# LioQing/wgpu-3dgs-core

Measured on AMD Instinct MI355X. Metric: Msplats/s @1080p (Gaussians per second through proj+sort+blend; 3 frames in flight on 3 priority streams), higher is better.
Workload: dtype f32; 1 GPU; 1M synthetic Gaussians, SH degree 0 (ShNone/RotScale 48 B), 1920x1080; gaussians=1000000, visible=708615, pairs=2550276, launches_per_frame=14, parallelism=single GPU, 3 frames in flight on 3 priority streams, frames_in_flight=3, renderer_scratch_copies=3

## Files before the change

### wgpu-3dgs-core_amd/csrc/gs_render_kernels.h

```cpp
#pragma once

#include <type_traits>

#include "gs_device_common.h"

namespace gs {

constexpr int PP_THREADS = 256;
constexpr int PP_ITEMS = 4;
constexpr int PP_CHUNK = PP_THREADS * PP_ITEMS;

struct FrameConsts {
    float M[16];
    float V[16];
    float ISR[9];
    float WS[9];
    float cam_pos[3];
    float fx, fy, cx, cy;
    float near_plane, far_plane;
    float size2, limx, limy, max_std_dev;
    float bg[3];
    uint32_t sh_deg, no_sh0;
    uint32_t width, height;
    uint32_t tiles_x, tiles_y;
// ... 2964 lines not shown
    if (wid == 0u) {
        blend_tile_range(tk, ranges, tile, lane, true, start, end);
        if (lane == 0u) {
            s_range[0] = start;
            s_range[1] = end;
        }
    }
    __syncthreads();
    start = s_range[0];
    end = s_range[1];
}

constexpr int BLEND_THREADS = 128;
constexpr int BLEND_BATCH = 128;

template <int MODE>
__global__ __launch_bounds__(BLEND_THREADS) void k_blend(uint32_t *__restrict__ ranges,
                                                         const uint32_t *__restrict__ idx,
                                                         const uint32_t *__restrict__ recs,
                                                         FrameConsts fc, float4 *__restrict__ rgba,
                                                         const FrameState *__restrict__ state, TileKeys tk) {
    if (state->overflow) return;
    __shared__ float4 s_a[2][BLEND_BATCH];
    __shared__ float4 s_b[2][BLEND_BATCH];
    __shared__ float2 s_c[2][BLEND_BATCH];
    __shared__ uint32_t s_cnt[2][2];
    __shared__ uint32_t s_alive[2];

    const uint32_t tid = threadIdx.x, lane = tid & 63u, wid = tid >> 6;
    const uint32_t tile = fc.band_ty0 * fc.tiles_x + blockIdx.x;
    const uint32_t ty = tile / fc.tiles_x, tx = tile % fc.tiles_x;
    const uint32_t px = tx * 16u + (lane & 15u);
    const uint32_t py0 = ty * 16u + wid * 8u + (lane >> 4), py1 = py0 + 4u;
    const float pxf = (float)px + 0.5f;
    const float rx0 = (float)(tx * 16u) + 0.5f, rx1 = rx0 + 15.0f;
    const float ry0 = (float)(ty * 16u) + 0.5f;

    uint32_t start, end;
    __shared__ uint32_t s_range[2];
    blend_tile_range_wg(tk, ranges, tile, lane, wid, s_range, start, end);
    f32x2 T = {1.0f, 1.0f}, C0 = {0.0f, 0.0f}, C1 = {0.0f, 0.0f}, C2 = {0.0f, 0.0f};
    const bool in0 = px < fc.width && py0 < fc.height, in1 = px < fc.width && py1 < fc.height;
    constexpr float DEAD = 1.0e15f;
    f32x2 pyf = {in0 ? (float)py0 + 0.5f : DEAD, in1 ? (float)py1 + 0.5f : DEAD};
    uint32_t remaining = __builtin_amdgcn_readfirstlane(
        (uint32_t)__popcll(__ballot(in0)) + (uint32_t)__popcll(__ballot(in1)));

    for (uint32_t b0 = start; b0 < end; b0 += BLEND_BATCH) {
        if (lane == 0) s_alive[wid] = remaining;
        __syncthreads();
        if ((s_alive[0] | s_alive[1]) == 0u) break;

        uint32_t j = b0 + tid;
        bool keep0 = false, keep1 = false;
        float pmin = 0.0f;
        u32x4_a4 r0, r1;
        uint32_t r2x = 0;
        if (j < end) {
            const uint32_t *rec = recs + (uint64_t)idx[j] * REC_WORDS;
            r0 = *(const u32x4_a4 *)(rec);
            r1 = *(const u32x4_a4 *)(rec + 4);
            r2x = rec[8];
            float mx = u2f(r0.x), my = u2f(r0.y), ca = u2f(r0.z), cb = u2f(r0.w), cc = u2f(r1.x);
            if constexpr (MODE == 0) {
                pmin = fmaxf(-__logf(255.0f * u2f(r1.y)) - 1.0e-3f, -5.6f);
                const float thr = (pmin - 0.1f) - cull_rounding_slack(mx, my, ca, cb, cc, rx0, ry0);
                keep0 = splat_touches_rect(mx, my, ca, cb, cc, rx0, rx1, ry0, ry0 + 7.0f, thr);
                keep1 = splat_touches_rect(mx, my, ca, cb, cc, rx0, rx1, ry0 + 8.0f, ry0 + 15.0f, thr);
            } else if constexpr (MODE == 1) {
                pmin = fc.ellipse_pmin;
                const float thr = (pmin - 0.1f - 1.0e-3f * fabsf(pmin)) - cull_rounding_slack(mx, my, ca, cb, cc, rx0, ry0);
                keep0 = splat_touches_rect(mx, my, ca, cb, cc, rx0, rx1, ry0, ry0 + 7.0f, thr);
                keep1 = splat_touches_rect(mx, my, ca, cb, cc, rx0, rx1, ry0 + 8.0f, ry0 + 15.0f, thr);
            } else {
                const float ex = mx - clampf(mx, rx0, rx1);
                const float ey0 = my - clampf(my, ry0, ry0 + 7.0f), ey1 = my - clampf(my, ry0 + 8.0f, ry0 + 15.0f);
                keep0 = ex * ex + ey0 * ey0 <= 2.26f;
                keep1 = ex * ex + ey1 * ey1 <= 2.26f;
            }
        }
        uint64_t m0 = __ballot(keep0), m1 = __ballot(keep1);
        if (lane == 0) {
            s_cnt[wid][0] = (uint32_t)__popcll(m0);
            s_cnt[wid][1] = (uint32_t)__popcll(m1);
        }
        __syncthreads();
        const uint32_t base0 = wid ? s_cnt[0][0] : 0u, base1 = wid ? s_cnt[0][1] : 0u;
        const uint32_t kept =
            __builtin_amdgcn_readfirstlane(s_cnt[0][wid] + s_cnt[1][wid]);
        if (keep0) {
            uint32_t pos = base0 + mbcnt(m0);
            s_a[0][pos] = make_float4(u2f(r0.x), u2f(r0.y), u2f(r0.z), u2f(r0.w));
            s_b[0][pos] = make_float4(u2f(r1.x), u2f(r1.y), u2f(r1.z), u2f(r1.w));
            s_c[0][pos] = make_float2(u2f(r2x), pmin);
        }
        if (keep1) {
            uint32_t pos = base1 + mbcnt(m1);
            s_a[1][pos] = make_float4(u2f(r0.x), u2f(r0.y), u2f(r0.z), u2f(r0.w));
            s_b[1][pos] = make_float4(u2f(r1.x), u2f(r1.y), u2f(r1.z), u2f(r1.w));
            s_c[1][pos] = make_float2(u2f(r2x), pmin);
        }
        __syncthreads();

        if (remaining != 0u) {
            for (uint32_t s = 0; s < kept; s++) {
                const float4 a = s_a[wid][s];
                const float4 bq = s_b[wid][s];
                const float dx = a.x - pxf;
                const f32x2 dy = f32x2{a.y, a.y} - pyf;
                const float u = a.z * dx, wq = a.w * dx;
                const f32x2 v = f32x2{bq.x, bq.x} * dy;
                f32x2 t = f32x2{wq, wq} * dy;
                t = pk_fma(v, dy, t);
                const f32x2 power = pk_fma(f32x2{u, u}, f32x2{dx, dx}, t);
                const float2 cq = s_c[wid][s];
                bool p0, p1;
                if constexpr (MODE == 2) {
                    const f32x2 d2 = f32x2{dx * dx, dx * dx} + dy * dy;
                    p0 = d2.x <= 2.25f;
                    p1 = d2.y <= 2.25f;
                } else {
                    p0 = power.x <= 0.0f && power.x >= cq.y;
                    p1 = power.y <= 0.0f && power.y >= cq.y;
                }
                if (!__any(p0 || p1)) continue;
                f32x2 alpha;
                if constexpr (MODE == 0) {
                const f32x2 tt = power * f32x2{1.44269504088896340736f, 1.44269504088896340736f};
                const f32x2 tm = tt + f32x2{12582912.0f, 12582912.0f};
                const f32x2 n = tm - f32x2{12582912.0f, 12582912.0f};
                const f32x2 f = tt - n;
                f32x2 p = {0x1.5f0896p-10f, 0x1.5f0896p-10f};
                p = pk_fma(p, f, f32x2{0x1.3cbf6cp-7f, 0x1.3cbf6cp-7f});
                p = pk_fma(p, f, f32x2{0x1.c6af6cp-5f, 0x1.c6af6cp-5f});
                p = pk_fma(p, f, f32x2{0x1.ebfa4ap-3f, 0x1.ebfa4ap-3f});
                p = pk_fma(p, f, f32x2{0x1.62e430p-1f, 0x1.62e430p-1f});
                p = pk_fma(p, f, f32x2{1.0f, 1.0f});
                const f32x2 e = {u2f(f2u(p.x) + (f2u(tm.x) << 23)), u2f(f2u(p.y) + (f2u(tm.y) << 23))};
                const f32x2 oe = f32x2{bq.y, bq.y} * e;
                alpha = f32x2{fminf(0.99f, oe.x), fminf(0.99f, oe.y)};
                } else {
                    const float flat = fminf(0.99f, bq.y);
                    alpha = f32x2{flat, flat};
                }
                const bool act0 = p0 && alpha.x >= (1.0f / 255.0f);
                const bool act1 = p1 && alpha.y >= (1.0f / 255.0f);
                f32x2 alpha_eff = {act0 ? alpha.x : 0.0f, act1 ? alpha.y : 0.0f};
                f32x2 test_T = T * (f32x2{1.0f, 1.0f} - alpha_eff);
                const bool fin0 = act0 && test_T.x < 0.0001f, fin1 = act1 && test_T.y < 0.0001f;
                if (__any(fin0 || fin1)) {
                    if (fin0) { pyf.x = DEAD; alpha_eff.x = 0.0f; test_T.x = T.x; }
                    if (fin1) { pyf.y = DEAD; alpha_eff.y = 0.0f; test_T.y = T.y; }
                    remaining = __builtin_amdgcn_readfirstlane(
                        remaining - ((uint32_t)__popcll(__ballot(fin0)) + (uint32_t)__popcll(__ballot(fin1))));
                }
                const f32x2 wgt = alpha_eff * T;
                C0 = pk_fma(f32x2{bq.z, bq.z}, wgt, C0);
                C1 = pk_fma(f32x2{bq.w, bq.w}, wgt, C1);
                C2 = pk_fma(f32x2{cq.x, cq.x}, wgt, C2);
                T = test_T;
                if (remaining == 0u) break;
            }
        }
    }
    if (in0) {
        float4 o;
        o.x = __builtin_fmaf(T.x, fc.bg[0], C0.x);
        o.y = __builtin_fmaf(T.x, fc.bg[1], C1.x);
        o.z = __builtin_fmaf(T.x, fc.bg[2], C2.x);
        o.w = 1.0f - T.x;
        store16(rgba + (uint64_t)py0 * fc.width + px, make_uint4(f2u(o.x), f2u(o.y), f2u(o.z), f2u(o.w)), fc.wt_stores);
    }
    if (in1) {
        float4 o;
        o.x = __builtin_fmaf(T.y, fc.bg[0], C0.y);
        o.y = __builtin_fmaf(T.y, fc.bg[1], C1.y);
        o.z = __builtin_fmaf(T.y, fc.bg[2], C2.y);
        o.w = 1.0f - T.y;
        store16(rgba + (uint64_t)py1 * fc.width + px, make_uint4(f2u(o.x), f2u(o.y), f2u(o.z), f2u(o.w)), fc.wt_stores);
    }
}


__device__ __forceinline__ bool splat_touches_rect2(float mx, float my, float ca, float cb, float cc,
                                                    float rx0, float rx1, float ry0, float ry1, float thr) {
    const float dx_lo = mx - rx1, dx_hi = mx - rx0, dy_lo = my - ry1, dy_hi = my - ry0;
    const bool in_x = dx_lo <= 0.0f && dx_hi >= 0.0f, in_y = dy_lo <= 0.0f && dy_hi >= 0.0f;
    const float dxn = fabsf(dx_lo) < fabsf(dx_hi) ? dx_lo : dx_hi;
    const float dyn = fabsf(dy_lo) < fabsf(dy_hi) ? dy_lo : dy_hi;
    const float mv = parabola_max(cc, cb * dxn, ca * dxn * dxn, dy_lo, dy_hi);
    const float mh = parabola_max(ca, cb * dyn, cc * dyn * dyn, dx_lo, dx_hi);
    return (in_x && in_y) || !(fmaxf(mv, mh) < thr);
}

constexpr uint32_t PICK_NONE = 0xffffffffu;
struct AuxIO {
    float *depth;
    uint32_t *pick;
    float tcut;
    uint32_t key_bias;
    const uint32_t *depth_keys;
    const uint32_t *block_list;
    const uint32_t *order;
};
__device__ __forceinline__ uint32_t aux_caller_index(const AuxIO &aux, uint32_t slot) {
    if (slot == PICK_NONE) return PICK_NONE;
    if (aux.block_list) slot = aux.block_list[slot / (uint32_t)PP_CHUNK] * (uint32_t)PP_CHUNK + slot % (uint32_t)PP_CHUNK;
    return aux.order ? aux.order[slot] : slot;
}
__device__ __forceinline__ void store4(void *p, uint32_t v, uint32_t mode) {
    if (mode == 1u) asm volatile("global_store_dword %0, %1, off sc1" ::"v"(p), "v"(v) : "memory");
    else if (mode == 2u) asm volatile("global_store_dword %0, %1, off nt" ::"v"(p), "v"(v) : "memory");
    else if (mode == 3u) asm volatile("global_store_dword %0, %1, off sc0 sc1" ::"v"(p), "v"(v) : "memory");
    else *(uint32_t *)p = v;
}
__device__ __forceinline__ void aux_store(const AuxIO &aux, uint64_t pix, uint32_t depth_bits, uint32_t pick, uint32_t mode) {
    if (aux.depth) store4(aux.depth + pix, depth_bits, mode);
    if (aux.pick) store4(aux.pick + pix, pick, mode);
}

__device__ __forceinline__ AuxIO aux_io() { return AuxIO{}; }
__device__ __forceinline__ AuxIO aux_io(AuxIO a) { return a; }

struct ContribIO {
    uint4 *rec;
    const uint32_t *block_list;
    const uint32_t *order;
};
__device__ __forceinline__ AuxIO aux_io(ContribIO) { return AuxIO{}; }
__device__ __forceinline__ ContribIO contrib_io() { return ContribIO{}; }
__device__ __forceinline__ ContribIO contrib_io(AuxIO) { return ContribIO{}; }
__device__ __forceinline__ ContribIO contrib_io(ContribIO c) { return c; }
template <typename... A> struct is_contrib_pack : std::false_type {};
template <> struct is_contrib_pack<ContribIO> : std::true_type {};
__device__ __forceinline__ uint32_t contrib_caller_index(const ContribIO &c, uint32_t slot) {
    if (c.block_list) slot = c.block_list[slot / (uint32_t)PP_CHUNK] * (uint32_t)PP_CHUNK + slot % (uint32_t)PP_CHUNK;
    return c.order ? c.order[slot] : slot;
}
template <int OFF> __device__ __forceinline__ uint32_t contrib_other_half(uint32_t v) {
    static_assert(OFF == 1 || OFF == 2 || OFF == 4 || OFF == 8 || OFF == 16, "inside a group of at most 32 lanes");
    if constexpr (OFF == 1) return (uint32_t)__builtin_amdgcn_update_dpp(0, (int)v, 0xB1, 0xf, 0xf, true);
    else if constexpr (OFF == 2) return (uint32_t)__builtin_amdgcn_update_dpp(0, (int)v, 0x4E, 0xf, 0xf, true);
    else if constexpr (OFF == 4) return (uint32_t)__builtin_amdgcn_update_dpp(0, (int)v, 0x141, 0xf, 0xf, true);
    else if constexpr (OFF == 8) return (uint32_t)__builtin_amdgcn_update_dpp(0, (int)v, 0x140, 0xf, 0xf, true);
    else return (uint32_t)__builtin_amdgcn_ds_swizzle((int)v, 0x401F);
}
template <int GL>
__device__ __forceinline__ void contrib_add(unsigned long long *s_qh, uint32_t *s_max, uint32_t acc, float w0, float w1, uint32_t lg) {
    uint32_t q = (uint32_t)(w0 * 16777216.0f) + (uint32_t)(w1 * 16777216.0f);
    uint32_t h = (w0 > 0.0f ? 1u : 0u) + (w1 > 0.0f ? 1u : 0u);
    uint32_t m = f2u(w0) > f2u(w1) ? f2u(w0) : f2u(w1);
#define GS_CONTRIB_FOLD(OFF)                                  \
    if constexpr (GL > OFF) {                                 \
        const uint32_t oq = contrib_other_half<OFF>(q);       \
        const uint32_t oh = contrib_other_half<OFF>(h);       \
        const uint32_t om = contrib_other_half<OFF>(m);       \
        q += oq;                                              \
        h += oh;                                              \
        m = om > m ? om : m;                                  \
    }
    GS_CONTRIB_FOLD(1)
    GS_CONTRIB_FOLD(2)
    GS_CONTRIB_FOLD(4)
    GS_CONTRIB_FOLD(8)
    GS_CONTRIB_FOLD(16)
#undef GS_CONTRIB_FOLD
    if (lg == 0u && h != 0u) {
        (void)__hip_atomic_fetch_add((unsigned long long *)((char *)s_qh + 2u * acc), ((unsigned long long)h << 32) | q, __ATOMIC_RELAXED,
                                     __HIP_MEMORY_SCOPE_WORKGROUP);
        (void)__hip_atomic_fetch_max((uint32_t *)((char *)s_max + acc), m, __ATOMIC_RELAXED, __HIP_MEMORY_SCOPE_WORKGROUP);
    }
}
__device__ __forceinline__ void contrib_flush(const ContribIO &c, uint32_t index, unsigned long long qh, uint32_t m) {
    if ((uint32_t)(qh >> 32) != 0u) {
        uint4 *p = c.rec + index;
        (void)__hip_atomic_fetch_add((unsigned long long *)p, qh & 0xffffffffull, __ATOMIC_RELAXED, __HIP_MEMORY_SCOPE_AGENT);
        (void)__hip_atomic_fetch_add((uint32_t *)p + 2, (uint32_t)(qh >> 32), __ATOMIC_RELAXED, __HIP_MEMORY_SCOPE_AGENT);
        (void)__hip_atomic_fetch_max((uint32_t *)p + 3, m, __ATOMIC_RELAXED, __HIP_MEMORY_SCOPE_AGENT);
    }
}

template <int MODE, int G, bool ROUNDS = false, bool AUX = false, typename... AuxArg>
__global__ __launch_bounds__(BLEND_THREADS) void k_blend_grouped(uint32_t *__restrict__ ranges,
                                                                 const uint32_t *__restrict__ idx,
                                                                 const uint32_t *__restrict__ recs,
                                                                 FrameConsts fc, float4 *__restrict__ rgba,
                                                                 const FrameState *__restrict__ state, TileKeys tk,
                                                                 AuxArg... aux_arg) {
    constexpr bool CONTRIB = is_contrib_pack<AuxArg...>::value;
    static_assert(sizeof...(AuxArg) == (AUX || CONTRIB ? 1u : 0u), "the AUX blend takes one AuxIO, the CONTRIB one one ContribIO, the plain one none");
    static_assert(!CONTRIB || (!AUX && !ROUNDS), "contribution frames take one round and no planes");
    static_assert(G == 2 || G == 4 || G == 8, "lane groups per wave");
    if (state->overflow) return;
    constexpr int GL = WAVE / G;
    constexpr int BW = G == 8 ? 4 : 8;
    constexpr int BH = 2 * GL / BW;
    constexpr int NCOL = 16 / BW;
    constexpr int NROW = 16 / BH;
    constexpr int NL = 2 * G;
    static_assert(NCOL * NROW == NL && G == NCOL * (NROW / 2), "one list per block, G blocks per wave");
    constexpr uint32_t NULL_REC = BLEND_BATCH;
    constexpr uint32_t RS = 48;
    __shared__ __attribute__((aligned(16))) float s_rec[(BLEND_BATCH + 1) * (RS / 4)];
    __shared__ __attribute__((aligned(16))) uint16_t s_list_mem[NL * BLEND_BATCH + (G == 8 ? 2 : 0)];
    uint16_t(*const s_list)[BLEND_BATCH] = (uint16_t(*)[BLEND_BATCH])s_list_mem;
    typedef typename std::conditional<G == 8, uint16_t, uint32_t>::type cnt_t;
    __shared__ __attribute__((aligned(16))) cnt_t s_cnt[2][NL];
    __shared__ uint32_t s_alive[2];

    const uint32_t tid = threadIdx.x, lane = tid & 63u, wid = tid >> 6;
    const uint32_t tile = fc.band_ty0 * fc.tiles_x + blockIdx.x;
    const uint32_t ty = tile / fc.tiles_x, tx = tile % fc.tiles_x;
    const uint32_t gi = lane / GL, lg = lane % GL;
    const uint32_t bx = gi % (uint32_t)NCOL, by = gi / (uint32_t)NCOL;
    const uint32_t px = tx * 16u + bx * (uint32_t)BW + lg % (uint32_t)BW;
    const uint32_t py0 = ty * 16u + wid * 8u + by * BH + lg / (uint32_t)BW, py1 = py0 + BH / 2;
    const float pxf = (float)px + 0.5f;
    const uint32_t my_list = wid * G + gi;
    const float tx0 = (float)(tx * 16u) + 0.5f, ty0 = (float)(ty * 16u) + 0.5f;

    if (ROUNDS && tk.round == 2u && ((tk.done[tile >> 5] >> (tile & 31u)) & 1u)) return;
    uint32_t start, end;
    __shared__ uint32_t s_range[2];
    __shared__ uint32_t s_limit[MODE == 0 ? 256 : 1];
    if constexpr (MODE == 0) {
        s_limit[tid] = k_blend_np_limit[tid];
        s_limit[tid + BLEND_THREADS] = k_blend_np_limit[tid + BLEND_THREADS];
    }
    blend_tile_range_wg(tk, ranges, tile, lane, wid, s_range, start, end);
    f32x2 T = {1.0f, 1.0f}, C0 = {0.0f, 0.0f}, C1 = {0.0f, 0.0f}, C2 = {0.0f, 0.0f};
    const bool in0 = px < fc.width && py0 < fc.height, in1 = px < fc.width && py1 < fc.height;
    constexpr float DEAD = 1.0e15f;
    bool live0 = in0, live1 = in1;
    if (ROUNDS && tk.round == 2u) {
        if (in0) {
            const float4 s = rgba[(uint64_t)py0 * fc.width + px];
            C0.x = s.x; C1.x = s.y; C2.x = s.z; T.x = fabsf(s.w);
            live0 = s.w > 0.0f;
        }
        if (in1) {
            const float4 s = rgba[(uint64_t)py1 * fc.width + px];
            C0.y = s.x; C1.y = s.y; C2.y = s.z; T.y = fabsf(s.w);
            live1 = s.w > 0.0f;
        }
    }
    f32x2 D = {0.0f, 0.0f};
    uint32_t pk0 = PICK_NONE, pk1 = PICK_NONE;
    const AuxIO aux = aux_io(aux_arg...);
    const ContribIO cio = contrib_io(aux_arg...);
    unsigned long long *s_qh = nullptr;
    uint32_t *s_max = nullptr;
    uint32_t my_index = 0u;
    bool flush_pending = false;
    if constexpr (CONTRIB) {
        __shared__ __attribute__((aligned(8))) unsigned long long s_contrib_qh[BLEND_BATCH];
        __shared__ uint32_t s_contrib_max[BLEND_BATCH];
        s_qh = s_contrib_qh;
        s_max = s_contrib_max;
    }
    if (AUX && ROUNDS && tk.round == 2u) {
        if (in0) {
            if (aux.depth) D.x = aux.depth[(uint64_t)py0 * fc.width + px];
            if (aux.pick) pk0 = aux.pick[(uint64_t)py0 * fc.width + px];
        }
        if (in1) {
            if (aux.depth) D.y = aux.depth[(uint64_t)py1 * fc.width + px];
            if (aux.pick) pk1 = aux.pick[(uint64_t)py1 * fc.width + px];
        }
    }
    f32x2 pyf = {live0 ? (float)py0 + 0.5f : DEAD, live1 ? (float)py1 + 0.5f : DEAD};
    uint32_t remaining = __builtin_amdgcn_readfirstlane(
        (uint32_t)__popcll(__ballot(live0)) + (uint32_t)__popcll(__ballot(live1)));
    if (tid == 0) {
        *(float4 *)(s_rec + NULL_REC * (RS / 4)) = make_float4(0.0f, 0.0f, 0.0f, 0.0f);
        *(float4 *)(s_rec + NULL_REC * (RS / 4) + 4) = make_float4(0.0f, MODE == 2 ? 1.0f : 0.0f, 0.0f, 0.0f);
        if constexpr (AUX || CONTRIB) *(float4 *)(s_rec + NULL_REC * (RS / 4) + 8) = make_float4(0.0f, 0.0f, 0.0f, 0.0f);
        else *(float2 *)(s_rec + NULL_REC * (RS / 4) + 8) = make_float2(0.0f, 0.0f);
    }

    for (uint32_t b0 = start; b0 < end; b0 += BLEND_BATCH) {
        if (lane == 0) s_alive[wid] = remaining;
        __syncthreads();
        if constexpr (CONTRIB) {
            if (flush_pending) contrib_flush(cio, my_index, s_qh[tid], s_max[tid]);
            flush_pending = false;
        }
        if ((s_alive[0] | s_alive[1]) == 0u) break;

        if constexpr (G == 8) {
            uint4 *l128 = (uint4 *)&s_list[0][0];
            constexpr uint32_t fill = (NULL_REC * RS) * 0x00010001u;
#pragma unroll
            for (uint32_t q = 0; q < NL * BLEND_BATCH / 8; q += BLEND_THREADS) l128[q + tid] = make_uint4(fill, fill, fill, fill);
        } else {
            uint32_t *l32 = (uint32_t *)&s_list[0][0];
            constexpr uint32_t fill = (NULL_REC * RS) * 0x00010001u;
            for (uint32_t q = tid; q < NL * BLEND_BATCH / 2; q += BLEND_THREADS) l32[q] = fill;
        }
        const uint32_t j = b0 + tid;
        float mx = 0.0f, my = 0.0f, ca = 0.0f, cb = 0.0f, cc = 0.0f, thr = 0.0f;
        uint32_t limit = 0u;
        const bool have = j < end;
        const bool staging = __builtin_amdgcn_ballot_w64(have) != 0ull;
        if constexpr (CONTRIB) {
            s_qh[tid] = 0ull;
            s_max[tid] = 0u;
        }
        uint64_t m[NL];
        if (!staging) {
#pragma unroll
            for (int l = 0; l < NL; l++) m[l] = 0ull;
        } else {
            if (have) {
                const uint32_t slot = idx[j];
                const uint32_t *rec = recs + (uint64_t)slot * REC_WORDS;
                const u32x4_a4 r0 = *(const u32x4_a4 *)(rec);
                const u32x4_a4 r1 = *(const u32x4_a4 *)(rec + 4);
                const uint32_t r2x = rec[8];
                mx = u2f(r0.x); my = u2f(r0.y); ca = u2f(r0.z); cb = u2f(r0.w); cc = u2f(r1.x);
                float pmin;
                if constexpr (MODE == 0) {
                    limit = s_limit[(uint32_t)(255.0f * u2f(r1.y) + 0.5f) & 255u];
                    pmin = fminf(-u2f(limit - 1u), 0.0f);
                } else {
                    pmin = fc.ellipse_pmin;
                    limit = f2u(fabsf(pmin)) + 1u;
                }
                thr = (MODE == 0 ? pmin : pmin - 1.0e-3f * fabsf(pmin)) - cull_rounding_slack(mx, my, ca, cb, cc, tx0, ty0);
                *(float4 *)(s_rec + tid * (RS / 4)) = make_float4(mx, my, ca, cb);
                *(float4 *)(s_rec + tid * (RS / 4) + 4) = make_float4(cc, MODE == 2 ? pmin : u2f(limit), u2f(r1.y), u2f(r1.z));
                if constexpr (AUX)
                    *(float4 *)(s_rec + tid * (RS / 4) + 8) =
                        make_float4(u2f(r1.w), u2f(r2x), u2f(aux.depth_keys[slot] + aux.key_bias), u2f(slot));
                else if constexpr (CONTRIB) {
                    *(float4 *)(s_rec + tid * (RS / 4) + 8) = make_float4(u2f(r1.w), u2f(r2x), 0.0f, u2f(tid * 4u));
                    my_index = contrib_caller_index(cio, slot);
                }
                else
                    *(float2 *)(s_rec + tid * (RS / 4) + 8) = make_float2(u2f(r1.w), u2f(r2x));
            }
            float bx0 = tx0, by0 = ty0;
            if constexpr (G == 8) asm volatile("" : "+v"(bx0), "+v"(by0));
            if constexpr (MODE == 2) {
#pragma unroll
                for (int l = 0; l < NL; l++) {
                    const int lw = l / G, lgi = l % G;
                    const float rx0 = bx0 + (float)BW * (float)(lgi % NCOL);
                    const float ry0 = by0 + 8.0f * (float)lw + (float)BH * (float)(lgi / NCOL);
                    const float ex = mx - clampf(mx, rx0, rx0 + (float)(BW - 1)), ey = my - clampf(my, ry0, ry0 + (float)(BH - 1));
                    m[l] = __builtin_amdgcn_ballot_w64(have && ex * ex + ey * ey <= 2.26f);
                }
            } else {
                const float rcc = __builtin_amdgcn_rcpf(cc), rca = __builtin_amdgcn_rcpf(ca);
                float c_lo[NCOL], c_hi[NCOL], c_q1[NCOL], c_q0[NCOL], c_t[NCOL];
                uint64_t c_inb[NCOL];
                const uint64_t have_b = __builtin_amdgcn_ballot_w64(have && limit != 0u);
#pragma unroll
                for (int c = 0; c < NCOL; c++) {
                    const float x0c = bx0 + (float)BW * (float)c;
                    c_lo[c] = mx - (x0c + (float)(BW - 1));
                    c_hi[c] = mx - x0c;
                    c_inb[c] = __builtin_amdgcn_ballot_w64(c_lo[c] <= 0.0f) & __builtin_amdgcn_ballot_w64(c_hi[c] >= 0.0f);
                    const float dn = fabsf(c_lo[c]) < fabsf(c_hi[c]) ? c_lo[c] : c_hi[c];
                    c_q1[c] = cb * dn;
                    c_q0[c] = ca * dn * dn;
                    c_t[c] = -0.5f * c_q1[c] * rcc;
                }
#pragma unroll
                for (int r = 0; r < NROW; r++) {
                    const float y0r = by0 + (float)(BH * r);
                    const float r_lo = my - (y0r + (float)(BH - 1)), r_hi = my - y0r;
                    const uint64_t r_inb = __builtin_amdgcn_ballot_w64(r_lo <= 0.0f) & __builtin_amdgcn_ballot_w64(r_hi >= 0.0f);
                    const float dn = fabsf(r_lo) < fabsf(r_hi) ? r_lo : r_hi;
                    const float r_q1 = cb * dn, r_q0 = cc * dn * dn;
                    const float r_t = -0.5f * r_q1 * rca;
#pragma unroll
                    for (int c = 0; c < NCOL; c++) {
                        const float tv = __builtin_amdgcn_fmed3f(c_t[c], r_lo, r_hi);
                        const float mv = __builtin_fmaf(__builtin_fmaf(cc, tv, c_q1[c]), tv, c_q0[c]);
                        const float th = __builtin_amdgcn_fmed3f(r_t, c_lo[c], c_hi[c]);
                        const float mh = __builtin_fmaf(__builtin_fmaf(ca, th, r_q1), th, r_q0);
                        const uint64_t keep = (c_inb[c] & r_inb) | __builtin_amdgcn_ballot_w64(!(fmaxf(mv, mh) < thr));
                        const int l = (r / (NROW / 2)) * G + (r % (NROW / 2)) * NCOL + c;
                        m[l] = keep & have_b;
                    }
                    if constexpr (G == 8) __builtin_amdgcn_sched_barrier(0);
                }
            }
        }
        if (lane == 0) {
            if constexpr (G == 8) {
                uint32_t *c32 = (uint32_t *)&s_cnt[wid][0];
#pragma unroll
                for (int l = 0; l < NL; l += 2) c32[l / 2] = (uint32_t)__popcll(m[l]) | ((uint32_t)__popcll(m[l + 1]) << 16);
            } else {
#pragma unroll
                for (int l = 0; l < NL; l++) s_cnt[wid][l] = (uint32_t)__popcll(m[l]);
            }
        }
        __syncthreads();
        if (!staging) {
        } else if constexpr (G == 8) {
            const uint4 *c128 = (const uint4 *)&s_cnt[0][0];
            const uint4 ca4 = c128[0], cb4 = c128[1];
            const uint32_t wv[8] = {ca4.x, ca4.y, ca4.z, ca4.w, cb4.x, cb4.y, cb4.z, cb4.w};
            uint32_t w[8];
#pragma unroll
            for (int q = 0; q < 8; q++) w[q] = (uint32_t)__builtin_amdgcn_readfirstlane(wv[q]);
            const uint32_t swid = (uint32_t)__builtin_amdgcn_readfirstlane(wid);
            const uint32_t dump = (uint32_t)(NL * BLEND_BATCH * sizeof(uint16_t));
#pragma unroll
            for (int l = 0; l < NL; l++) {
                const uint32_t base = swid ? (w[l / 2] >> (16 * (l & 1))) & 0xffffu : 0u;
                const uint32_t pos = __builtin_amdgcn_mbcnt_hi((uint32_t)(m[l] >> 32), __builtin_amdgcn_mbcnt_lo((uint32_t)m[l], 0u));
                const uint32_t at = (pos << 1) + 2u * ((uint32_t)(l * BLEND_BATCH) + base);
                uint32_t to;
                asm("v_cndmask_b32 %0, %1, %2, %3" : "=v"(to) : "v"(dump), "v"(at), "s"(m[l]));
                *(uint16_t *)((char *)s_list_mem + to) = (uint16_t)(tid * RS);
            }
        } else {
            uint32_t lbase[NL];
#pragma unroll
            for (int l = 0; l < NL; l++) lbase[l] = s_cnt[0][l];
            __builtin_amdgcn_sched_barrier(0);
#pragma unroll
            for (int l = 0; l < NL; l++)
                if ((m[l] >> lane) & 1ull) s_list[l][(wid ? lbase[l] : 0u) + mbcnt(m[l])] = (uint16_t)(tid * RS);
        }
        uint32_t trip = 0;
        if constexpr (G == 8) {
            const uint4 c0 = *(const uint4 *)&s_cnt[0][wid * G], c1 = *(const uint4 *)&s_cnt[1][wid * G];
            const uint32_t sum[4] = {c0.x + c1.x, c0.y + c1.y, c0.z + c1.z, c0.w + c1.w};
#pragma unroll
            for (int q = 0; q < 4; q++) {
                const uint32_t lo = sum[q] & 0xffffu, hi = sum[q] >> 16;
                trip = lo > trip ? lo : trip;
                trip = hi > trip ? hi : trip;
            }
        } else {
#pragma unroll
            for (int g = 0; g < G; g++) {
                const uint32_t c = s_cnt[0][wid * G + g] + s_cnt[1][wid * G + g];
                trip = c > trip ? c : trip;
            }
        }
        trip = __builtin_amdgcn_readfirstlane(trip);
        __syncthreads();

        if (remaining != 0u) {
            const uint32_t *mine = (const uint32_t *)s_list[my_list];
            const char *rbase = (const char *)s_rec;
            const uint32_t trips = (trip + 1u) >> 1;
            uint32_t pair = mine[0];
            uint32_t id_A = pair & 0xffffu;
            float4 a_A = *(const float4 *)(rbase + id_A), b_A = *(const float4 *)(rbase + id_A + 16);
#define GS_BLEND_STEP(AREC, BREC, ID)                                                                         \
    {                                                                                                         \
        const float dx = AREC.x - pxf;                                                                        \
        const f32x2 dy = f32x2{AREC.y, AREC.y} - pyf;                                                         \
        const float u = -(AREC.z * dx), wq = -(AREC.w * dx);                                                  \
        const f32x2 v = -(f32x2{BREC.x, BREC.x} * dy);                                                        \
        f32x2 t = f32x2{wq, wq} * dy;                                                                         \
        t = pk_fma(v, dy, t);                                                                                 \
                                                                  \
        const f32x2 np = pk_fma(f32x2{u, u}, f32x2{dx, dx}, t);                                               \
        bool p0, p1;                                                                                          \
        if constexpr (MODE == 2) {                                                                            \
            const f32x2 d2 = f32x2{dx * dx, dx * dx} + dy * dy;                                               \
            p0 = d2.x <= 2.25f && BREC.y <= 0.0f;                       \
            p1 = d2.y <= 2.25f && BREC.y <= 0.0f;                                                             \
        } else {                                                                                              \
            p0 = f2u(np.x) < f2u(BREC.y);                                    \
            p1 = f2u(np.y) < f2u(BREC.y);                                                                     \
        }                                                                                                     \
        if (__builtin_amdgcn_ballot_w64(p0 || p1) != 0ull) {                                                  \
            float2 cq;                                                                              \
            float zq = 0.0f;                                   \
            uint32_t sq = 0u;                                                                                 \
            if constexpr (AUX || CONTRIB) {                                                                   \
                const float4 c4 = *(const float4 *)(rbase + ID + 32);                                         \
                cq = make_float2(c4.x, c4.y);                                                                 \
                zq = c4.z;                                                                                    \
                sq = f2u(c4.w);                                                                               \
            } else {                                                                                          \
                cq = *(const float2 *)(rbase + ID + 32);                                                      \
            }                                                                                                 \
            f32x2 alpha;                                                                                      \
            if constexpr (MODE == 0) {                                                                        \
                                                              \
                const f32x2 tt = np * f32x2{-1.44269504088896340736f, -1.44269504088896340736f};              \
                const f32x2 tm = tt + f32x2{12582912.0f, 12582912.0f};                                        \
                const f32x2 n = tm - f32x2{12582912.0f, 12582912.0f};                                         \
                const f32x2 f = tt - n;                                                                       \
                f32x2 p = {0x1.5f0896p-10f, 0x1.5f0896p-10f};                                                 \
                p = pk_fma(p, f, f32x2{0x1.3cbf6cp-7f, 0x1.3cbf6cp-7f});                                      \
                p = pk_fma(p, f, f32x2{0x1.c6af6cp-5f, 0x1.c6af6cp-5f});                                      \
                p = pk_fma(p, f, f32x2{0x1.ebfa4ap-3f, 0x1.ebfa4ap-3f});                                      \
                p = pk_fma(p, f, f32x2{0x1.62e430p-1f, 0x1.62e430p-1f});                                      \
                p = pk_fma(p, f, f32x2{1.0f, 1.0f});                                                          \
                const f32x2 e = {u2f(f2u(p.x) + (f2u(tm.x) << 23)), u2f(f2u(p.y) + (f2u(tm.y) << 23))};       \
                const f32x2 oe = f32x2{BREC.z, BREC.z} * e;                                                   \
                alpha = f32x2{fminf(0.99f, oe.x), fminf(0.99f, oe.y)};                                        \
            } else {                                                                                          \
                const float flat = fminf(0.99f, BREC.z);                                                      \
                alpha = f32x2{flat, flat};                                                                    \
            }                                                                                                 \
                \
            const bool act0 = p0 && (MODE == 0 || alpha.x >= (1.0f / 255.0f));                                \
            const bool act1 = p1 && (MODE == 0 || alpha.y >= (1.0f / 255.0f));                                \
                              \
                                    \
            f32x2 alpha_eff = {act0 ? alpha.x : 0.0f, act1 ? alpha.y : 0.0f};                                 \
            f32x2 test_T = T * (f32x2{1.0f, 1.0f} - alpha_eff);                                               \
                 \
                                                                 \
            const bool fin0 = test_T.x < 0.0001f, fin1 = test_T.y < 0.0001f;                                  \
            const uint64_t f0 = __builtin_amdgcn_ballot_w64(fin0), f1 = __builtin_amdgcn_ballot_w64(fin1);    \
            if ((f0 | f1) != 0ull) {                  \
                if (fin0) { pyf.x = DEAD; alpha_eff.x = 0.0f; test_T.x = T.x; }                               \
                if (fin1) { pyf.y = DEAD; alpha_eff.y = 0.0f; test_T.y = T.y; }                               \
                remaining -= (uint32_t)__popcll(f0) + (uint32_t)__popcll(f1);                                 \
            }                                                                                                 \
            const f32x2 wgt = alpha_eff * T;                                                                  \
            C0 = pk_fma(f32x2{BREC.w, BREC.w}, wgt, C0);                                                      \
            C1 = pk_fma(f32x2{cq.x, cq.x}, wgt, C1);                                                          \
            C2 = pk_fma(f32x2{cq.y, cq.y}, wgt, C2);                                                          \
            if constexpr (AUX) {                                                                              \
                D = pk_fma(f32x2{zq, zq}, wgt, D);                                                            \
                pk0 = alpha_eff.x > 0.0f && T.x > aux.tcut ? sq : pk0;                                        \
                pk1 = alpha_eff.y > 0.0f && T.y > aux.tcut ? sq : pk1;                                        \
            }                                                                                                 \
            if constexpr (CONTRIB) {   \
                if (__builtin_amdgcn_ballot_w64(wgt.x > 0.0f || wgt.y > 0.0f) != 0ull)                        \
                    contrib_add<GL>(s_qh, s_max, sq, wgt.x, wgt.y, lg);                                       \
            }                                                                                                 \
            T = test_T;                                                                                       \
        }                                                                                                     \
    }
            for (uint32_t q = 0; q < trips && remaining != 0u; q++) {
                const uint32_t id_B = pair >> 16;
                const float4 a_B = *(const float4 *)(rbase + id_B), b_B = *(const float4 *)(rbase + id_B + 16);
                pair = mine[q + 1 < (uint32_t)(BLEND_BATCH / 2) ? q + 1 : q];
                GS_BLEND_STEP(a_A, b_A, id_A)
                id_A = pair & 0xffffu;
                a_A = *(const float4 *)(rbase + id_A);
                b_A = *(const float4 *)(rbase + id_A + 16);
                GS_BLEND_STEP(a_B, b_B, id_B)
            }
#undef GS_BLEND_STEP
        }
        if constexpr (CONTRIB) flush_pending = true;
    }
    if constexpr (CONTRIB) {
        if (flush_pending) {
            __syncthreads();
            contrib_flush(cio, my_index, s_qh[tid], s_max[tid]);
        }
    }
    if (ROUNDS && tk.round == 1u) {
        if (lane == 0) s_alive[wid] = remaining;
        __syncthreads();
        if ((s_alive[0] | s_alive[1]) != 0u) {
            if (in0)
                store16(rgba + (uint64_t)py0 * fc.width + px,
                        make_uint4(f2u(C0.x), f2u(C1.x), f2u(C2.x), f2u(pyf.x == DEAD ? -T.x : T.x)), fc.wt_stores);
            if (in1)
                store16(rgba + (uint64_t)py1 * fc.width + px,
                        make_uint4(f2u(C0.y), f2u(C1.y), f2u(C2.y), f2u(pyf.y == DEAD ? -T.y : T.y)), fc.wt_stores);
            if constexpr (AUX) {
                if (in0) aux_store(aux, (uint64_t)py0 * fc.width + px, f2u(D.x), pk0, fc.wt_stores);
                if (in1) aux_store(aux, (uint64_t)py1 * fc.width + px, f2u(D.y), pk1, fc.wt_stores);
            }
            if (tid == 0 && end > start) atomicOr(tk.open + (tile >> 5), 1u << (tile & 31u));
            return;
        }
        if (tid == 0) atomicOr(tk.done + (tile >> 5), 1u << (tile & 31u));
    }
    if (in0) {
        float4 o;
        o.x = __builtin_fmaf(T.x, fc.bg[0], C0.x);
        o.y = __builtin_fmaf(T.x, fc.bg[1], C1.x);
        o.z = __builtin_fmaf(T.x, fc.bg[2], C2.x);
        o.w = 1.0f - T.x;
        store16(rgba + (uint64_t)py0 * fc.width + px, make_uint4(f2u(o.x), f2u(o.y), f2u(o.z), f2u(o.w)), fc.wt_stores);
    }
    if (in1) {
        float4 o;
        o.x = __builtin_fmaf(T.y, fc.bg[0], C0.y);
        o.y = __builtin_fmaf(T.y, fc.bg[1], C1.y);
        o.z = __builtin_fmaf(T.y, fc.bg[2], C2.y);
        o.w = 1.0f - T.y;
        store16(rgba + (uint64_t)py1 * fc.width + px, make_uint4(f2u(o.x), f2u(o.y), f2u(o.z), f2u(o.w)), fc.wt_stores);
    }
    if constexpr (AUX) {
        if (in0) aux_store(aux, (uint64_t)py0 * fc.width + px, f2u(D.x), T.x > aux.tcut ? PICK_NONE : aux_caller_index(aux, pk0), fc.wt_stores);
        if (in1) aux_store(aux, (uint64_t)py1 * fc.width + px, f2u(D.y), T.y > aux.tcut ? PICK_NONE : aux_caller_index(aux, pk1), fc.wt_stores);
    }
}


struct VisibleIO {
    const uint32_t *depth;
    const uint32_t *chunk_vis;
    const uint32_t *recs;
    const uint32_t *block_list;
    const uint32_t *list_blocks;
    const uint32_t *order;
    uint32_t n, nslots;
    float x0, y0, x1, y1;
    const uint8_t *mask;
    uint32_t width, height;
    uint32_t *scratch;
};

__global__ __launch_bounds__(256) void k_select_visible(VisibleIO io) {
    const uint32_t slot = blockIdx.x * 256u + threadIdx.x;
    const uint32_t limit = io.block_list ? *io.list_blocks * (uint32_t)PP_CHUNK : io.nslots;
    if (slot >= limit || slot >= io.nslots) return;
    if (io.chunk_vis[slot / (uint32_t)PP_CHUNK] == 0u || io.depth[slot] == 0xffffffffu) return;
    const float mx = u2f(io.recs[(uint64_t)slot * REC_WORDS]), my = u2f(io.recs[(uint64_t)slot * REC_WORDS + 1u]);
    if (!(io.x0 <= mx && mx < io.x1 && io.y0 <= my && my < io.y1)) return;
    if (io.mask) {
        if (!(mx >= 0.0f && my >= 0.0f && mx < (float)io.width && my < (float)io.height)) return;
        const uint32_t px = (uint32_t)floorf(mx), py = (uint32_t)floorf(my);
        if (px >= io.width || py >= io.height || io.mask[(uint64_t)py * io.width + px] == 0u) return;
    }
    uint32_t ms = slot;
    if (io.block_list) ms = io.block_list[slot / (uint32_t)PP_CHUNK] * (uint32_t)PP_CHUNK + slot % (uint32_t)PP_CHUNK;
    if (ms >= io.n) return;
    const uint32_t i = io.order ? io.order[ms] : ms;
    if (i >= io.n) return;
    atomicOr(&io.scratch[i >> 5], 1u << (i & 31u));
}

__global__ __launch_bounds__(PP_THREADS) void k_selection_to_slots(const uint32_t *__restrict__ words,
                                                                   const uint32_t *__restrict__ order, uint32_t n,
                                                                   uint64_t *__restrict__ out,
                                                                   uint32_t *__restrict__ block_hidden) {
    __shared__ uint32_t s_all[PP_THREADS / WAVE];
    const uint32_t lane = threadIdx.x & 63u, wid = threadIdx.x >> 6;
    bool all = true;
#pragma unroll
    for (int k = 0; k < PP_ITEMS; k++) {
        const uint32_t slot = blockIdx.x * (uint32_t)PP_CHUNK + k * PP_THREADS + threadIdx.x;
        bool bit = false;
        if (slot < n) {
            const uint32_t i = order ? order[slot] : slot;
            bit = i < n && ((words[i >> 5] >> (i & 31u)) & 1u);
        }
        const uint64_t m = __ballot(bit), valid = __ballot(slot < n);
        if (lane == 0u) out[slot >> 6] = m;
        all = all && m == valid;
    }
    if (!block_hidden) return;
    if (lane == 0u) s_all[wid] = all ? 1u : 0u;
    __syncthreads();
    if (threadIdx.x == 0u) block_hidden[blockIdx.x] = (s_all[0] & s_all[1]) & (s_all[2] & s_all[3]);
}
}
```

Measured before the change: 4813 Msplats/s.

## Reorder blend record layout and software-pipeline LDS loads inside the blend step

Reorders the fields of the per-gaussian shared-memory record so the values the coverage test needs first sit together. The blend loop is unrolled to four records per iteration, and the next record's LDS load is issued in the middle of the current step, after the coverage predicate and before the ballot. A padded sentinel list entry is added so the look-ahead read past the end of a list stays safe. The aim is to hide LDS latency in the blend inner loop, at the cost of more registers and more code.

```diff
diff --git a/wgpu-3dgs-core_amd/csrc/gs_render_kernels.h b/wgpu-3dgs-core_amd/csrc/gs_render_kernels.h
--- a/wgpu-3dgs-core_amd/csrc/gs_render_kernels.h
+++ b/wgpu-3dgs-core_amd/csrc/gs_render_kernels.h
@@ -3290,7 +3290,8 @@
     constexpr uint32_t NULL_REC = BLEND_BATCH;
     constexpr uint32_t RS = 48;
     __shared__ __attribute__((aligned(16))) float s_rec[(BLEND_BATCH + 1) * (RS / 4)];
-    __shared__ __attribute__((aligned(16))) uint16_t s_list_mem[NL * BLEND_BATCH + (G == 8 ? 2 : 0)];
+    constexpr int LIST_PAD = 2;
+    __shared__ __attribute__((aligned(16))) uint16_t s_list_mem[NL * BLEND_BATCH + LIST_PAD + (G == 8 ? 2 : 0)];
     uint16_t(*const s_list)[BLEND_BATCH] = (uint16_t(*)[BLEND_BATCH])s_list_mem;
     typedef typename std::conditional<G == 8, uint16_t, uint32_t>::type cnt_t;
     __shared__ __attribute__((aligned(16))) cnt_t s_cnt[2][NL];
@@ -3361,9 +3362,11 @@
         (uint32_t)__popcll(__ballot(live0)) + (uint32_t)__popcll(__ballot(live1)));
     if (tid == 0) {
         *(float4 *)(s_rec + NULL_REC * (RS / 4)) = make_float4(0.0f, 0.0f, 0.0f, 0.0f);
-        *(float4 *)(s_rec + NULL_REC * (RS / 4) + 4) = make_float4(0.0f, MODE == 2 ? 1.0f : 0.0f, 0.0f, 0.0f);
+        *(float4 *)(s_rec + NULL_REC * (RS / 4) + 4) = make_float4(0.0f, 0.0f, 0.0f, MODE == 2 ? 1.0f : 0.0f);
         if constexpr (AUX || CONTRIB) *(float4 *)(s_rec + NULL_REC * (RS / 4) + 8) = make_float4(0.0f, 0.0f, 0.0f, 0.0f);
         else *(float2 *)(s_rec + NULL_REC * (RS / 4) + 8) = make_float2(0.0f, 0.0f);
+        static_assert(LIST_PAD == 2, "the pad is one 32-bit store");
+        *(uint32_t *)(s_list_mem + NL * BLEND_BATCH) = (NULL_REC * RS) * 0x00010001u;
     }
 
     for (uint32_t b0 = start; b0 < end; b0 += BLEND_BATCH) {
@@ -3414,9 +3417,10 @@
                     pmin = fc.ellipse_pmin;
                     limit = f2u(fabsf(pmin)) + 1u;
                 }
+                *(float4 *)(s_rec + tid * (RS / 4)) = make_float4(my, mx, cc, ca);
+                *(float4 *)(s_rec + tid * (RS / 4) + 4) = make_float4(u2f(r1.y), cb, u2f(r1.z), MODE == 2 ? pmin : u2f(limit));
+                __builtin_amdgcn_sched_barrier(0);
                 thr = (MODE == 0 ? pmin : pmin - 1.0e-3f * fabsf(pmin)) - cull_rounding_slack(mx, my, ca, cb, cc, tx0, ty0);
-                *(float4 *)(s_rec + tid * (RS / 4)) = make_float4(mx, my, ca, cb);
-                *(float4 *)(s_rec + tid * (RS / 4) + 4) = make_float4(cc, MODE == 2 ? pmin : u2f(limit), u2f(r1.y), u2f(r1.z));
                 if constexpr (AUX)
                     *(float4 *)(s_rec + tid * (RS / 4) + 8) =
                         make_float4(u2f(r1.w), u2f(r2x), u2f(aux.depth_keys[slot] + aux.key_bias), u2f(slot));
@@ -3496,7 +3500,7 @@
 #pragma unroll
             for (int q = 0; q < 8; q++) w[q] = (uint32_t)__builtin_amdgcn_readfirstlane(wv[q]);
             const uint32_t swid = (uint32_t)__builtin_amdgcn_readfirstlane(wid);
-            const uint32_t dump = (uint32_t)(NL * BLEND_BATCH * sizeof(uint16_t));
+            const uint32_t dump = (uint32_t)((NL * BLEND_BATCH + LIST_PAD) * sizeof(uint16_t));
 #pragma unroll
             for (int l = 0; l < NL; l++) {
                 const uint32_t base = swid ? (w[l / 2] >> (16 * (l & 1))) & 0xffffu : 0u;
@@ -3536,18 +3540,17 @@
         __syncthreads();
 
         if (remaining != 0u) {
-            const uint32_t *mine = (const uint32_t *)s_list[my_list];
+            const char *lp = (const char *)s_list[my_list];
             const char *rbase = (const char *)s_rec;
-            const uint32_t trips = (trip + 1u) >> 1;
-            uint32_t pair = mine[0];
-            uint32_t id_A = pair & 0xffffu;
-            float4 a_A = *(const float4 *)(rbase + id_A), b_A = *(const float4 *)(rbase + id_A + 16);
-#define GS_BLEND_STEP(AREC, BREC, ID)                                                                         \
+            const uint32_t trips = (trip + 1u) >> 1, quads = trips >> 1;
+            uint32_t id_A = *(const uint32_t *)lp & 0xffffu, id_B;
+            float4 a_A = *(const float4 *)(rbase + id_A), b_A = *(const float4 *)(rbase + id_A + 16), a_B, b_B;
+#define GS_BLEND_STEP(AREC, BREC, ID, NEXT)                                                                   \
     {                                                                                                         \
-        const float dx = AREC.x - pxf;                                                                        \
-        const f32x2 dy = f32x2{AREC.y, AREC.y} - pyf;                                                         \
-        const float u = -(AREC.z * dx), wq = -(AREC.w * dx);                                                  \
-        const f32x2 v = -(f32x2{BREC.x, BREC.x} * dy);                                                        \
+        const float dx = AREC.y - pxf;                                                                        \
+        const f32x2 dy = f32x2{AREC.x, AREC.x} - pyf;                                                         \
+        const float u = -(AREC.w * dx), wq = -(BREC.y * dx);                                                  \
+        const f32x2 v = -(f32x2{AREC.z, AREC.z} * dy);                                                        \
         f32x2 t = f32x2{wq, wq} * dy;                                                                         \
         t = pk_fma(v, dy, t);                                                                                 \
                                                                   \
@@ -3555,12 +3558,13 @@
         bool p0, p1;                                                                                          \
         if constexpr (MODE == 2) {                                                                            \
             const f32x2 d2 = f32x2{dx * dx, dx * dx} + dy * dy;                                               \
-            p0 = d2.x <= 2.25f && BREC.y <= 0.0f;                       \
-            p1 = d2.y <= 2.25f && BREC.y <= 0.0f;                                                             \
+            p0 = d2.x <= 2.25f && BREC.w <= 0.0f;                       \
+            p1 = d2.y <= 2.25f && BREC.w <= 0.0f;                                                             \
         } else {                                                                                              \
-            p0 = f2u(np.x) < f2u(BREC.y);                                    \
-            p1 = f2u(np.y) < f2u(BREC.y);                                                                     \
+            p0 = f2u(np.x) < f2u(BREC.w);                                    \
+            p1 = f2u(np.y) < f2u(BREC.w);                                                                     \
         }                                                                                                     \
+        NEXT                                                                     \
         if (__builtin_amdgcn_ballot_w64(p0 || p1) != 0ull) {                                                  \
             float2 cq;                                                                              \
             float zq = 0.0f;                                   \
@@ -3587,10 +3591,10 @@
                 p = pk_fma(p, f, f32x2{0x1.62e430p-1f, 0x1.62e430p-1f});                                      \
                 p = pk_fma(p, f, f32x2{1.0f, 1.0f});                                                          \
                 const f32x2 e = {u2f(f2u(p.x) + (f2u(tm.x) << 23)), u2f(f2u(p.y) + (f2u(tm.y) << 23))};       \
-                const f32x2 oe = f32x2{BREC.z, BREC.z} * e;                                                   \
+                const f32x2 oe = f32x2{BREC.x, BREC.x} * e;                                                   \
                 alpha = f32x2{fminf(0.99f, oe.x), fminf(0.99f, oe.y)};                                        \
             } else {                                                                                          \
-                const float flat = fminf(0.99f, BREC.z);                                                      \
+                const float flat = fminf(0.99f, BREC.x);                                                      \
                 alpha = f32x2{flat, flat};                                                                    \
             }                                                                                                 \
                 \
@@ -3610,7 +3614,7 @@
                 remaining -= (uint32_t)__popcll(f0) + (uint32_t)__popcll(f1);                                 \
             }                                                                                                 \
             const f32x2 wgt = alpha_eff * T;                                                                  \
-            C0 = pk_fma(f32x2{BREC.w, BREC.w}, wgt, C0);                                                      \
+            C0 = pk_fma(f32x2{BREC.z, BREC.z}, wgt, C0);                                                      \
             C1 = pk_fma(f32x2{cq.x, cq.x}, wgt, C1);                                                          \
             C2 = pk_fma(f32x2{cq.y, cq.y}, wgt, C2);                                                          \
             if constexpr (AUX) {                                                                              \
@@ -3625,16 +3629,28 @@
             T = test_T;                                                                                       \
         }                                                                                                     \
     }
-            for (uint32_t q = 0; q < trips && remaining != 0u; q++) {
-                const uint32_t id_B = pair >> 16;
-                const float4 a_B = *(const float4 *)(rbase + id_B), b_B = *(const float4 *)(rbase + id_B + 16);
-                pair = mine[q + 1 < (uint32_t)(BLEND_BATCH / 2) ? q + 1 : q];
-                GS_BLEND_STEP(a_A, b_A, id_A)
-                id_A = pair & 0xffffu;
-                a_A = *(const float4 *)(rbase + id_A);
-                b_A = *(const float4 *)(rbase + id_A + 16);
-                GS_BLEND_STEP(a_B, b_B, id_B)
-            }
+#define GS_LIST_ID(K) ((uint32_t) * (const uint16_t *)(lp + 2 * (K)))
+#define GS_LOAD_REC(R)                             \
+    a_##R = *(const float4 *)(rbase + id_##R);     \
+    b_##R = *(const float4 *)(rbase + id_##R + 16);
+            for (uint32_t q = 0; q < quads && remaining != 0u; q++) {
+                id_B = GS_LIST_ID(1);
+                GS_BLEND_STEP(a_A, b_A, id_A, GS_LOAD_REC(B))
+                id_A = GS_LIST_ID(2);
+                GS_BLEND_STEP(a_B, b_B, id_B, GS_LOAD_REC(A))
+                id_B = GS_LIST_ID(3);
+                GS_BLEND_STEP(a_A, b_A, id_A, GS_LOAD_REC(B))
+                id_A = GS_LIST_ID(4);
+                GS_BLEND_STEP(a_B, b_B, id_B, GS_LOAD_REC(A))
+                lp += 8;
+            }
+            if ((trips & 1u) != 0u && remaining != 0u) {
+                id_B = GS_LIST_ID(1);
+                GS_BLEND_STEP(a_A, b_A, id_A, GS_LOAD_REC(B))
+                GS_BLEND_STEP(a_B, b_B, id_B, )
+            }
+#undef GS_LOAD_REC
+#undef GS_LIST_ID
 #undef GS_BLEND_STEP
         }
         if constexpr (CONTRIB) flush_pending = true;
```

Measured after the change: 4878 Msplats/s (median of 6 runs). +1.4%, better.
